# MihailMihov/simd-raytracer

Measured on AMD Instinct MI355X. Metric: Mrays/s (intersect invocations per second), hw09/scene5 dragon 1920x1080 1spp, higher is better.
Workload: dtype f32; 1 GPU; BASELINE configs[1]: scenes/hw09/scene5.crtscene 1920x1080 1spp max_ray_depth=5 (primary + shadow + reflection rays), kd_tree_simd_accel semantics; rays_per_frame=2726485, primary_rays=2073600, parallelism=bucket-tiles x1

## Files before the change

simd-raytracer_amd/csrc/accel.hpp:

```cpp
#pragma once

#include <hip/hip_runtime.h>

#include <cstdlib>
#include <mutex>
#include <string>
#include <vector>

#include "abi_guard.hpp"
#include "kernels.hpp"
#include "stream.hpp"
#include "build.hpp"
#include "dev_mem.hpp"
#include "frame_plan.hpp"
#include "update_plan.hpp"

struct rtk_knobs {
    uint32_t slice_min_tris = rtk::kSliceMinTrisDefault;
    bool shadow_exit = true;
    bool skip_unlit_shadow = true;
    bool bundle_cull = true;
    bool auto_trials = true;
    bool cost_feedback = true;
    unsigned resort_every = 16;
    uint32_t light_cycles = 140000u;
    uint32_t order_floor_cycles = 20000u;
    bool batch_scalar_surv = false;
    bool stream_scalar_surv = true;
    bool repack = true;
    bool raster_tiles = true;
    int repack_skip_bits = 6;
    bool repack_full_bounds = false;
    int repack_skip_bits2 = 14;
    bool repack_dirs3 = false;
    int repack_trace = -1;
    size_t group8_below = 9000;
    int stream_node_factor = 0;
    int stream_deep_level = 99, stream_deep_mode = RTK_TRACE_AUTO;
    uint32_t auto_min_lanes = 12;
    int stream_sort_from = -1;
    bool stream_debug = false;
    bool stream_side = true;
    int stream_lanes = 4;
    int stream_slices = 0;
    int stream_batch = 0;
    int stream_mem_gb = 96;
    int stream_side_below = 2;
    bool first_frame_prior = true;
    bool fast_occluders = true;
    bool camera_keeps_order = false;
    size_t views_launch_units = 131072;
    bool traversal_fast = false;
    size_t adaptive_chunk_pixels = size_t(1) << 20;

    static rtk_knobs from_env() {
        rtk_knobs k;
        auto geti = [](const char *name, long &out) { const char *e = std::getenv(name); if (!e || !*e) return false; out = std::atol(e); return true; };
        long v;
        if (geti("RTK_SLICE_MIN_TRIS", v) && v > 0) k.slice_min_tris = uint32_t(v);
        if (geti("RTK_SHADOW_EARLY_EXIT", v)) k.shadow_exit = v != 0;
        if (geti("RTK_SKIP_UNLIT_SHADOW", v)) k.skip_unlit_shadow = v != 0;
        if (geti("RTK_BUNDLE_CULL", v)) k.bundle_cull = v != 0;
        if (geti("RTK_AUTO_TRIALS", v)) k.auto_trials = v != 0;
        if (geti("RTK_COST_FEEDBACK", v)) k.cost_feedback = v != 0;
        if (geti("RTK_COST_RESORT_EVERY", v) && v > 0) k.resort_every = unsigned(v);
        if (geti("RTK_LIGHT_BELOW_CYCLES", v) && v >= 0) k.light_cycles = uint32_t(v);
        if (geti("RTK_ORDER_FLOOR_CYCLES", v) && v >= 0) k.order_floor_cycles = uint32_t(v);
        if (geti("RTK_REPACK", v)) k.repack = v != 0;
        if (geti("RTK_RASTER_TILES", v)) k.raster_tiles = v != 0;
        if (geti("RTK_REPACK_FULL_BOUNDS", v)) k.repack_full_bounds = v != 0;
        if (geti("RTK_REPACK_SKIP_BITS2", v) && v >= 0 && v <= 22) k.repack_skip_bits2 = int(v);
        if (geti("RTK_REPACK_DIRS3", v)) k.repack_dirs3 = v != 0;
        if (geti("RTK_REPACK_SKIP_BITS", v) && v >= 0 && v <= 14) k.repack_skip_bits = int(v);
        if (geti("RTK_STREAM_SCALAR_SURV", v)) k.stream_scalar_surv = v != 0;
        if (geti("RTK_BATCH_SCALAR_SURV", v)) k.batch_scalar_surv = v != 0;
        if (geti("RTK_REPACK_TRACE", v) && (v == RTK_TRACE_AUTO || v == RTK_TRACE_WAVE || v == RTK_TRACE_LANE)) k.repack_trace = int(v);
        if (geti("RTK_GROUP8_BELOW_BLOCKS", v) && v >= 0) k.group8_below = size_t(v);
        if (geti("RTK_STREAM_NODE_FACTOR", v) && v >= 1) k.stream_node_factor = int(v);
        if (geti("RTK_STREAM_DEEP_LEVEL", v)) k.stream_deep_level = int(v);
        if (geti("RTK_STREAM_DEEP_MODE", v)) k.stream_deep_mode = int(v);
        if (geti("RTK_AUTO_MIN_LANES", v) && v > 0 && v <= 64) k.auto_min_lanes = uint32_t(v);
        if (geti("RTK_STREAM_SORT_FROM", v)) k.stream_sort_from = int(v);
        if (geti("RTK_STREAM_DEBUG", v)) k.stream_debug = v != 0;
        if (geti("RTK_STREAM_SIDE", v)) k.stream_side = v != 0;
        if (geti("RTK_TRAVERSAL_FAST", v)) k.traversal_fast = v != 0;
        if (geti("RTK_FIRST_FRAME_PRIOR", v)) k.first_frame_prior = v != 0;
        if (geti("RTK_STREAM_SLICES", v) && (v == 0 || v == 1 || v == 2 || v == 4)) k.stream_slices = int(v);
        if (geti("RTK_STREAM_BATCH", v) && v >= 0 && v <= 4096) k.stream_batch = int(v);
        if (geti("RTK_STREAM_MEM_GB", v) && v >= 1 && v <= 256) k.stream_mem_gb = int(v);
        if (geti("RTK_FAST_OCCLUDERS", v)) k.fast_occluders = v != 0;
        if (geti("RTK_STREAM_SIDE_BELOW", v) && v >= 0) k.stream_side_below = int(v);
        if (geti("RTK_VIEWS_LAUNCH_UNITS", v) && v >= 1 && v <= (1l << 30)) k.views_launch_units = size_t(v);
        if (geti("RTK_CAMERA_KEEPS_ORDER", v)) k.camera_keeps_order = v != 0;
        if (geti("RTK_STREAM_LANES", v) && v >= 1 && v <= rtk::dev::kStreamLanes) k.stream_lanes = int(v);
        if (geti("RTK_ADAPTIVE_CHUNK_PIXELS", v) && v >= 1 && v <= (1l << 30)) k.adaptive_chunk_pixels = size_t(v);
        return k;
    }
};
// ... 246 lines not shown
    if (src.empty()) return RTK_OK;
    const hipError_t e = hipMemcpy(dst.get(), src.data(), src.size() * sizeof(T), hipMemcpyHostToDevice);
    if (e != hipSuccess) { dst.reset(); return hip_fail(e, "upload"); }
    return RTK_OK;
}

inline bool valid_mode(int m) { return m == RTK_TRACE_AUTO || m == RTK_TRACE_LANE || m == RTK_TRACE_WAVE; }
inline bool valid_batch_mode(int m) { return valid_mode(m) || m == RTK_TRACE_REPACK; }
inline bool valid_frame_mode(int m) { return valid_mode(m) || m == RTK_TRACE_GROUP4 || m == RTK_TRACE_GROUP8 || m == RTK_TRACE_GROUP16 ||
           m == RTK_TRACE_STREAM || m == RTK_TRACE_TWOPASS; }

inline int stream_slices_for(const HostTree &t) {
    double refs = 0.0, sq = 0.0;
    for (const DevNode &l : t.dev_leaves) { refs += double(l.b); sq += double(l.b) * double(l.b); }
    return (refs > 0.0 && sq / refs < 150.0) ? 1 : 4;
}

inline bool scene_forks(const rtk_accel *a, int diffuse_rays) { return a->has_refractive || diffuse_rays > 0; }
inline bool scene_general(const rtk_accel *a, int diffuse_rays) { return scene_forks(a, diffuse_rays) || !a->scene.textures.empty(); }

inline unsigned long long *counters_now(const rtk_accel *a) { return a->d_counters.get() + size_t(a->cnt.current) * kCounterAllocWords; }
inline unsigned long long *counters_other(const rtk_accel *a) { return a->d_counters.get() + size_t(a->cnt.current ^ 1) * kCounterAllocWords; }

int ensure_device(rtk_accel *a, hipStream_t s = nullptr);
dev::TreeView tree_view(const rtk_accel *a);
enum : unsigned { kKeepViewOrders = 1u, kKeepTrial = 2u };
inline void forget_orders(rtk_accel *a, unsigned keep = 0u) {
    a->fb.forget();
    a->cnt.forget();
    if (!(keep & kKeepViewOrders)) for (rtk_cost_feedback &f : a->fb_views) f.forget();
    for (rtk_cost_feedback &f : a->fb_regions) f.forget();
    if (!(keep & kKeepTrial)) a->trial.abandon();
}

int remake_occluders(rtk_accel *a, const std::vector<DevMaterial> &materials, const DevMaterial *d_materials, hipStream_t s);
int ensure_update_static(rtk_accel *a);
void dense_texture_slots(rtk_accel *a);
const std::vector<float> &host_vert_uv(rtk_accel *a);
int ensure_vert_uv_dev(rtk_accel *a);
int frame_geom(const rtk_accel *a, const rtk_render_params *p, FrameGeom &g);
rtk_view accel_camera(const rtk_accel *a);
void camera_args(const rtk_view &cam, const rtk_render_params *p, const FrameGeom &g, dev::RenderArgs &A);
int ensure_stream_ws(rtk_accel *a, size_t pixels, size_t nodes, size_t lights, bool need_sum, int lanes);
hipError_t zero_counters(rtk_accel *a, hipStream_t s);
void record_last(rtk_accel *a, hipStream_t s, bool stats, uint64_t primary);
int radiance_device_impl(rtk_accel *a, const rtk_ray *d_rays, const uint32_t *d_ids, size_t n, const rtk_radiance_params *p,
                         float *d_rgb, hipStream_t s, uint32_t *n_chunks_out);
void free_stream_ws(rtk_accel *a);
struct StreamSetup {
    dev::StreamArgs S;
    int deep_level, deep_mode, sort_from, slices;
    size_t factor, node_bytes, budget;
};
StreamSetup stream_args(const rtk_accel *a, const dev::RenderArgs &A, int diffuse_rays, bool forks);
int claim_stream_ws(rtk_accel *a, hipStream_t s);
int release_stream_ws(rtk_accel *a, hipStream_t s);
int fork_lanes(rtk_accel *a, int lanes, hipStream_t s);
int join_lanes(rtk_accel *a, int lanes, hipStream_t s);
dev::RenderArgs frame_args(const rtk_accel *a, const rtk_render_params *p, const FrameGeom &g, const rtk_view &cam, float *d_out);
int adaptive_device_impl(rtk_accel *a, const rtk_render_params *p, const rtk_adaptive_params *ap, const FrameGeom &g, float *d_rgb,
                         uint32_t *d_samples, float *d_noise, hipStream_t s);

}
```

simd-raytracer_amd/csrc/api_frame.hip:

```cpp
#include <cmath>
#include <cstdio>
#include <cstring>
#include <mutex>

#include "accel.hpp"
#include "stream_plan.hpp"

namespace rtk {

int frame_geom(const rtk_accel *a, const rtk_render_params *p, FrameGeom &g) {
    if (!a || !p) return fail(RTK_ERR_INVALID, "null accel or params");
    const int64_t w = p->width > 0 ? p->width : a->scene.width;
    const int64_t h = p->height > 0 ? p->height : a->scene.height;
    if (w <= 0 || h <= 0 || w > 65536 || h > 65536) return fail(RTK_ERR_INVALID, "image size must be in [1, 65536]");
    if (p->spp < 1) return fail(RTK_ERR_INVALID, "spp must be >= 1");
    if (p->max_ray_depth < 0 || p->max_ray_depth > kMaxRayDepth)
        return fail(RTK_ERR_INVALID, "max_ray_depth must be in [0, 16]");
    if (p->diffuse_rays < 0 || p->diffuse_rays > 32767) return fail(RTK_ERR_INVALID, "diffuse_rays must be in [0, 32767]");
    if (!valid_frame_mode(p->trace_mode)) return fail(RTK_ERR_INVALID, "unknown trace_mode");
    if (p->sample_begin < 0 || p->sample_count < 0 || p->sample_begin >= p->spp ||
        int64_t(p->sample_begin) + p->sample_count > p->spp)
        return fail(RTK_ERR_INVALID, "sample_begin / sample_count must select samples inside [0, spp)");
    if (p->sample_count == 0 && p->sample_begin != 0) return fail(RTK_ERR_INVALID, "sample_count == 0 means all samples: sample_begin must be 0");
    g.sample_begin = p->sample_begin;
// ... 283 lines not shown
    RTK_MEM(fb.cost.reserve(cap));
    RTK_MEM(fb.order.reserve(2 * (2 * cap + 4) + 8));
    RTK_MEM(fb.bins.reserve(cap));
    fb.state.units = cap;
    return RTK_OK;
}

struct ListSet { uint32_t *order, *hdr, *wg_list; };
ListSet list_set(rtk_cost_feedback &fb, int k, size_t units) {
    uint32_t *const order = fb.order.get() + size_t(k) * (2 * fb.state.units + 4);
    return {order, order + units, order + units + 4};
}

int launch_sort(rtk_accel *a, rtk_cost_feedback &fb, int k, int frame_mode, size_t units, hipStream_t s) {
    const ListSet L = list_set(fb, k, units);
    RTK_HIP_AS(launch_order_by_cost(fb.cost.get(), fb.bins.get(), L.order, L.wg_list, L.hdr, uint32_t(units),
                                    frame_mode == RTK_TRACE_GROUP4 ? a->knobs.light_cycles >> 4 : 0u, a->knobs.order_floor_cycles >> 4, 4u, s),
               "launch k_order_by_cost");
    RTK_MEM(fb.nwgs_host.reserve(1));
    RTK_MEM(fb.nwgs_ev.ensure());
    RTK_HIP(hipMemcpyAsync(fb.nwgs_host.get(), L.hdr, sizeof(uint32_t), hipMemcpyDeviceToHost, s));
    RTK_HIP(hipEventRecord(fb.nwgs_ev.get(), s));
    return RTK_OK;
}

int order_launch(rtk_accel *a, rtk_cost_feedback &fb, const rtk_render_params *p, const FrameGeom &g, dev::RenderArgs &A, int frame_mode,
                 size_t units, hipStream_t s, OrderState::Step &step) {
    uint64_t sig[5];
    shape_sig(g, p->spp, p->max_ray_depth, p->diffuse_rays, sig);
    sig[3] = (uint64_t(uint32_t(g.bucket)) << 32) | (uint64_t(uint32_t(g.sample_end - g.sample_begin) & 0xFFFFu) << 16) | uint32_t(p->trace_mode);
    sig[4] = A.regions ? ((1ull << 63) | (uint64_t(A.n_regions) << 32) | uint64_t(A.n_units))
                       : (A.views ? uint64_t(A.n_views) : 0ull);
    RTK_TRY(ensure_feedback_ws(a, fb, g, units));
    step = fb.state.step(sig, frame_mode, p->collect_stats != 0, A.regions != nullptr, {a->knobs.first_frame_prior, a->knobs.resort_every});
    const ListSet L = list_set(fb, step.read_set, units);
    if (step.prior)
        RTK_HIP_AS(launch_block_prior(A, fb.bins.get(), L.order, L.wg_list, L.hdr,
                                      reinterpret_cast<uint32_t *>(A.counters + kPriorScratchWord), 4u, s), "launch k_block_prior");
    if (step.sort_front) RTK_TRY(launch_sort(a, fb, step.read_set, frame_mode, units, s));
    if (step.use_order) { A.order_in = L.order; A.order_hdr = L.hdr; A.wg_list = L.wg_list; }
    if (&fb == &a->fb) a->cnt.after_order(step);
    A.cost_out = fb.cost.get();
    return RTK_OK;
}

int render_megakernel(rtk_accel *a, rtk_cost_feedback &fb, const rtk_render_params *p, const FrameGeom &g, dev::RenderArgs &A, bool general,
                      hipStream_t s) {
    const size_t units = A.regions ? size_t(A.n_units) : (A.views ? g.blocks() * A.n_views : g.blocks());
    A.n_units = uint32_t(units);
    const int frame_mode = OrderState::frame_mode(p->trace_mode, units, a->knobs.group8_below);
    OrderState::Step step = {};
    if (a->knobs.cost_feedback && units > 0 && units <= 0x7FFFFFFFull) {
        const int rc = order_launch(a, fb, p, g, A, frame_mode, units, s, step);
        if (rc != RTK_OK) { fb.forget(); return rc; }
    }
    unsigned n_wgs = 0;
    if (A.wg_list != nullptr) {
        bool ready = false;
        if (fb.state.awaits_count() && !(ready = hipEventQuery(fb.nwgs_ev.get()) == hipSuccess)) (void)hipGetLastError();
        n_wgs = fb.state.workgroups(ready, fb.nwgs_host.get());
    }
    int rc = RTK_OK;
    const hipError_t e = launch_render(A, frame_mode, p->collect_stats != 0, general, s, n_wgs);
    if (e != hipSuccess) rc = hip_fail(e, "launch k_render");
    if (rc == RTK_OK && step.sort_behind) rc = launch_sort(a, fb, step.write_set, frame_mode, units, s);
    if (rc != RTK_OK) fb.forget();
    return rc;
}

}

dev::RenderArgs frame_args(const rtk_accel *a, const rtk_render_params *p, const FrameGeom &g, const rtk_view &cam, float *d_out) {
    dev::RenderArgs A = scene_args(a, p->collect_stats);
    camera_args(cam, p, g, A);
    A.max_depth = p->max_ray_depth; A.diffuse_rays = p->diffuse_rays;
// ... 416 lines not shown
        if (ids) RTK_HIP(hipMemcpy(a->rad_ids.get(), ids, n * sizeof(uint32_t), hipMemcpyHostToDevice));
        uint32_t n_chunks = 0;
        RTK_TRY(radiance_device_impl(a, a->rad_rays.get(), ids ? a->rad_ids.get() : nullptr, n, p, a->rad_rgb.get(), nullptr, &n_chunks));
        RTK_HIP(hipMemcpy(rgb, a->rad_rgb.get(), n * 3 * sizeof(float), hipMemcpyDeviceToHost));
        unsigned long long h[kRadianceTotalWords] = {};
        RTK_HIP(hipMemcpy(h, a->d_rad_counters.get() + radiance_total_word(dev::kStreamLanes), sizeof(h), hipMemcpyDeviceToHost));
        if (counters) {
            std::memset(counters, 0, sizeof(*counters));
            counters->rays = h[kRadianceRays]; counters->primary = n;
        }
        if (a->knobs.stream_debug)
            std::fprintf(stderr, "[rtk radiance] rays %zu chunks %u redone %llu node_cap %u\n", n, n_chunks, h[kRadianceRedone], a->ws.node_cap);
        return RTK_OK;
    });
}


int rtk_accel_get_camera(const rtk_accel *a, rtk_view *out) {
    return abi_guard([&]() -> int {
        if (!a || !out) return fail(RTK_ERR_INVALID, "null accel or view");
        std::lock_guard<std::mutex> lock(const_cast<rtk_accel *>(a)->mu);
        *out = accel_camera(a);
        return RTK_OK;
    });
}

int rtk_accel_set_camera(rtk_accel *a, const rtk_view *view) {
    return abi_guard([&]() -> int {
        if (!a || !view) return fail(RTK_ERR_INVALID, "null accel or view");
        std::lock_guard<std::mutex> lock(a->mu);
        std::memcpy(a->scene.cam_pos, view->position, sizeof(a->scene.cam_pos));
        std::memcpy(a->scene.cam_mat, view->matrix, sizeof(a->scene.cam_mat));
        if (!a->knobs.camera_keeps_order) forget_orders(a, kKeepViewOrders | kKeepTrial);
        return RTK_OK;
    });
}

int rtk_render_views_device(rtk_accel *a, const rtk_render_params *p, const rtk_view *d_views, int32_t n_views, float *d_out, void *stream) {
    return abi_guard([&]() -> int {
        if (!a || !p) return fail(RTK_ERR_INVALID, "null accel or params");
        FrameGeom g;
        RTK_TRY(views_check(a, p, d_views, n_views, d_out, g));
        if (n_views == 0) return RTK_OK;
        std::lock_guard<std::mutex> lock(a->mu);
        RTK_TRY(ensure_device(a, static_cast<hipStream_t>(stream)));
        return render_views_impl(a, p, g, nullptr, d_views, n_views, d_out, static_cast<hipStream_t>(stream));
    });
}

int rtk_render_views(rtk_accel *a, const rtk_render_params *p, const rtk_view *views, int32_t n_views, float *rgb, rtk_counters *counters) {
    return abi_guard([&]() -> int {
        if (!a || !p) return fail(RTK_ERR_INVALID, "null accel or params");
        FrameGeom g;
        RTK_TRY(views_check(a, p, views, n_views, rgb, g));
        if (n_views == 0) return RTK_OK;
        {
            std::lock_guard<std::mutex> lock(a->mu);
            RTK_TRY(ensure_device(a));
            const size_t n = size_t(n_views), nf = n * g.width * g.height * 3;
            RTK_MEM(a->views_tab.reserve(n));
            RTK_MEM(a->views_out.reserve(nf));
            RTK_HIP(hipMemcpy(a->views_tab.get(), views, n * sizeof(rtk_view), hipMemcpyHostToDevice));
            if (p->sample_begin > 0) RTK_HIP(hipMemcpy(a->views_out.get(), rgb, nf * sizeof(float), hipMemcpyHostToDevice));
            RTK_TRY(render_views_impl(a, p, g, views, a->views_tab.get(), n_views, a->views_out.get(), nullptr));
            RTK_HIP(hipMemcpy(rgb, a->views_out.get(), nf * sizeof(float), hipMemcpyDeviceToHost));
        }
// ... 79 lines not shown
```

simd-raytracer_amd/csrc/api_state.hip:

```cpp
#include <algorithm>
#include <cstring>
#include <mutex>

#include "accel.hpp"

using namespace rtk;

namespace {

int reserve_lights(rtk_accel *a, size_t n) {
    if (n <= a->d_lights.capacity()) return RTK_OK;
    DevBuf<DevLight> larger;
    RTK_MEM(larger.reserve(n, grow_lights()));
    a->d_lights.swap(larger);
    return RTK_OK;
}

void lights_changed(rtk_accel *a, size_t n_before) {
    if (a->scene.lights.size() == n_before) return;
    forget_orders(a, kKeepTrial);
}


constexpr size_t kTexelLimit = 0x7FFFFFFFull;
constexpr size_t kSlotAlign = 16;

inline size_t slot_round(size_t bytes) { return (bytes + kSlotAlign - 1) & ~(kSlotAlign - 1); }
inline bool is_bitmap(const DevTexture &t) { return t.kind == RTK_TEX_BITMAP; }
inline size_t texel_bytes(const DevTexture &t) { return is_bitmap(t) ? size_t(t.bmp[0]) * size_t(t.bmp[1]) * 3 : 0; }

inline bool bitmap_size_ok(int32_t w, int32_t h) { return w >= 1 && h >= 1 && int64_t(w) * int64_t(h) <= (int64_t{1} << 28); }

void host_tri_uv(const rtk_accel *a, const std::vector<float> &vert_uv, std::vector<DevTriUv> &out) {
    std::vector<size_t> first(a->mesh_nverts.size() + 1, 0);
    for (size_t mi = 0; mi < a->mesh_nverts.size(); ++mi) first[mi + 1] = first[mi] + size_t(a->mesh_nverts[mi]);
    out.resize(a->tree.triangles.size());
    for (size_t i = 0; i < out.size(); ++i) {
        const HostTriangle &tr = a->tree.triangles[i];
        for (int k = 0; k < 3; ++k) {
            const size_t g = first[tr.mesh] + tr.vi[k];
            out[i].uv[k * 2] = vert_uv[g * 2]; out[i].uv[k * 2 + 1] = vert_uv[g * 2 + 1];
        }
    }
}

int make_tri_uv(rtk_accel *a, hipStream_t s) {
    RTK_TRY(ensure_update_static(a));
    const size_t nt = size_t(a->scene.n_triangles);
    RTK_MEM(a->topo_spare.tri_uv.reserve(std::max<size_t>(1, nt), grow_bytes()));
    RTK_HIP_AS(launch_tri_uv(a->topo.index.get(), a->topo_vert_uv.get(), uint32_t(nt), uint32_t(a->scene.n_vertices), a->topo_spare.tri_uv.get(), s),
               "launch k_tri_uv");
    return RTK_OK;
// ... 67 lines not shown
struct HostTexels {
    bool same = false;
    std::vector<DevTexture> table;
    std::vector<uint8_t> pixels;
};
int host_texels(const rtk_accel *a, size_t texture, int32_t w, int32_t h, const uint8_t *rgb, HostTexels &H) {
    const std::vector<DevTexture> &tex = a->scene.textures;
    const size_t was = texel_bytes(tex[texture]), need = size_t(w) * size_t(h) * 3, at = size_t(tex[texture].bmp[2]);
    const std::vector<uint8_t> &old = a->scene.tex_pixels;
    if (old.size() - was + need > kTexelLimit) return fail(RTK_ERR_INVALID, "the texel bytes of all bitmaps must fit an int32 offset");
    H.same = tex[texture].bmp[0] == w && tex[texture].bmp[1] == h;
    if (H.same) return RTK_OK;
    H.table = tex;
    H.table[texture].bmp[0] = w; H.table[texture].bmp[1] = h;
    for (size_t i = 0; i < tex.size(); ++i)
        if (is_bitmap(tex[i]) && size_t(tex[i].bmp[2]) > at) H.table[i].bmp[2] = int32_t(size_t(tex[i].bmp[2]) - was + need);
    H.pixels.resize(old.size() - was + need);
    std::memcpy(H.pixels.data(), old.data(), at);
    if (rgb) std::memcpy(H.pixels.data() + at, rgb, need);
    std::memcpy(H.pixels.data() + at + need, old.data() + at + was, old.size() - at - was);
    return RTK_OK;
}

int check_texel_call(const rtk_accel *a, int32_t texture, int32_t w, int32_t h) {
    if (texture < 0 || size_t(texture) >= a->scene.textures.size()) return fail(RTK_ERR_INVALID, "texture index out of range");
    if (!bitmap_size_ok(w, h)) return fail(RTK_ERR_INVALID, "bad bitmap texture size");
    if (!is_bitmap(a->scene.textures[size_t(texture)])) return fail(RTK_ERR_INVALID, "the texture is not a bitmap");
    return RTK_OK;
}

void adopt_texels(rtk_accel *a, size_t texture, HostTexels &H, const uint8_t *rgb, TexelPlan *P, bool on_device) {
    if (H.same) { if (rgb) std::memcpy(a->scene.tex_pixels.data() + a->scene.textures[texture].bmp[2], rgb, texel_bytes(a->scene.textures[texture])); }
    else { a->scene.textures.swap(H.table); a->scene.tex_pixels.swap(H.pixels); }
    if (!P) return;
    if (P->moved) { a->d_tex_pixels.swap(a->tx_pixels); a->d_textures.swap(a->tx_textures); }
    a->tx_slots.swap(P->slots); a->tx_used = P->used;
    a->tx_slots[texture].on_device = on_device;
}

template <typename Write>
int set_texels_device(rtk_accel *a, int32_t texture, int32_t w, int32_t h, const void *d_src, hipStream_t s, Write write) {
    if (!a || !d_src) return fail(RTK_ERR_INVALID, "null accel or texels");
    std::lock_guard<std::mutex> lock(a->mu);
    RTK_TRY(check_texel_call(a, texture, w, h));
    HostTexels H;
    RTK_TRY(host_texels(a, size_t(texture), w, h, nullptr, H));
    RTK_TRY(ensure_device(a));
    RTK_HIP(a->geom_fence.quiesce());
    DevTexture row = a->scene.textures[size_t(texture)];
    row.bmp[0] = w; row.bmp[1] = h;
    TexelPlan P;
    RTK_TRY(place_texels(a, size_t(texture), row, size_t(w) * size_t(h) * 3, s, P));
    RTK_TRY(write(P.dst, s));
    RTK_HIP(a->geom_fence.publish(s));
    adopt_texels(a, size_t(texture), H, nullptr, &P, true);
    return RTK_OK;
}

}

void rtk::dense_texture_slots(rtk_accel *a) {
    const std::vector<DevTexture> &tex = a->scene.textures;
    a->tx_slots.assign(tex.size(), rtk_accel::TexSlot{});
    for (size_t i = 0; i < tex.size(); ++i)
        if (is_bitmap(tex[i])) { a->tx_slots[i].off = tex[i].bmp[2]; a->tx_slots[i].cap = texel_bytes(tex[i]); }
    a->tx_used = a->scene.tex_pixels.size();
// ... 106 lines not shown
                if (m.texture < 0 || size_t(m.texture) >= a->scene.textures.size()) return fail(RTK_ERR_INVALID, "texture material refers to a texture that does not exist");
            } else m.texture = -1;
            m.pad = 0u;
        }
        if (a->on_device) {
            RTK_HIP(hipSetDevice(a->device));
            RTK_HIP(a->geom_fence.quiesce());
            RTK_MEM(a->st_materials.reserve(table.size()));
            if (!table.empty()) RTK_HIP(hipMemcpy(a->st_materials.get(), table.data(), table.size() * sizeof(DevMaterial), hipMemcpyHostToDevice));
            RTK_TRY(remake_occluders(a, table, a->st_materials.get(), nullptr));
            a->d_materials.swap(a->st_materials);
        }
        a->scene.materials.swap(table);
        a->has_refractive = any_refractive(a->scene.materials);
        forget_orders(a);
        return RTK_OK;
    });
}

int rtk_accel_get_background(const rtk_accel *a, float rgb[3]) {
    return abi_guard([&]() -> int {
        if (!a || !rgb) return fail(RTK_ERR_INVALID, "null accel or colour");
        std::lock_guard<std::mutex> lock(const_cast<rtk_accel *>(a)->mu);
        std::memcpy(rgb, a->scene.background, sizeof(a->scene.background));
        return RTK_OK;
    });
}

int rtk_accel_set_background(rtk_accel *a, const float rgb[3]) {
    return abi_guard([&]() -> int {
        if (!a || !rgb) return fail(RTK_ERR_INVALID, "null accel or colour");
        std::lock_guard<std::mutex> lock(a->mu);
        std::memcpy(a->scene.background, rgb, sizeof(a->scene.background));
        return RTK_OK;
    });
}


int rtk_accel_get_textures(const rtk_accel *a, rtk_texture *out, int32_t cap, int32_t *n) {
    return abi_guard([&]() -> int {
        if (!a || !n) return fail(RTK_ERR_INVALID, "null accel or count");
        std::lock_guard<std::mutex> lock(const_cast<rtk_accel *>(a)->mu);
        const std::vector<DevTexture> &tex = a->scene.textures;
        *n = int32_t(tex.size());
        const size_t take = (out && cap > 0) ? std::min(tex.size(), size_t(cap)) : 0;
        for (size_t i = 0; i < take; ++i) {
            rtk_texture t{};
            t.kind = tex[i].kind;
            if (is_bitmap(tex[i])) { t.width = tex[i].bmp[0]; t.height = tex[i].bmp[1]; }
            else { std::memcpy(t.color_a, tex[i].a, sizeof(t.color_a)); std::memcpy(t.color_b, tex[i].b, sizeof(t.color_b)); t.param = tex[i].param; }
            out[i] = t;
        }
        return RTK_OK;
    });
}

int rtk_accel_get_texture_pixels(const rtk_accel *a, int32_t texture, uint8_t *out, size_t cap, size_t *n_bytes) {
    return abi_guard([&]() -> int {
        if (!a || !n_bytes) return fail(RTK_ERR_INVALID, "null accel or size");
        std::lock_guard<std::mutex> lock(const_cast<rtk_accel *>(a)->mu);
        if (texture < 0 || size_t(texture) >= a->scene.textures.size()) return fail(RTK_ERR_INVALID, "texture index out of range");
        const DevTexture &t = a->scene.textures[size_t(texture)];
        *n_bytes = texel_bytes(t);
        const size_t take = out ? std::min(*n_bytes, cap) : 0;
        if (take == 0) return RTK_OK;
        if (a->on_device && a->tx_slots[size_t(texture)].on_device) {
// ... 36 lines not shown
            if (is_bitmap(table[i])) std::memcpy(texels.data() + table[i].bmp[2], pixels[i], texel_bytes(table[i]));
        const bool first = a->scene.textures.empty() && !table.empty();
        std::vector<DevTriUv> tri_uv;
        std::vector<rtk_accel::TexSlot> slots(table.size());
        size_t used = 0;
        if (a->on_device) {
            RTK_HIP(hipSetDevice(a->device));
            RTK_HIP(a->geom_fence.quiesce());
            std::vector<DevTexture> rows(table.size());
            for (size_t i = 0; i < table.size(); ++i) {
                if (is_bitmap(table[i])) { slots[i].off = int32_t(used); slots[i].cap = slot_round(texel_bytes(table[i])); used += slots[i].cap; }
                if (used > kTexelLimit) return fail(RTK_ERR_INVALID, "the texel bytes of all bitmaps must fit an int32 offset");
                rows[i] = device_row(table[i], slots[i]);
            }
            RTK_MEM(a->tx_textures.reserve(std::max<size_t>(1, rows.size())));
            if (!rows.empty()) RTK_HIP(hipMemcpy(a->tx_textures.get(), rows.data(), rows.size() * sizeof(DevTexture), hipMemcpyHostToDevice));
            if (used > 0) RTK_MEM(a->tx_pixels.reserve(used, grow_bytes()));
            for (size_t i = 0; i < table.size(); ++i)
                if (is_bitmap(table[i])) RTK_HIP(hipMemcpy(a->tx_pixels.get() + slots[i].off, pixels[i], texel_bytes(table[i]), hipMemcpyHostToDevice));
            if (first) {
                RTK_TRY(ensure_vert_uv_dev(a));
                RTK_TRY(make_tri_uv(a, nullptr));
                RTK_HIP(a->geom_fence.publish(nullptr));
            }
        } else if (first) host_tri_uv(a, host_vert_uv(a), tri_uv);
        if (a->on_device) {
            a->d_textures.swap(a->tx_textures);
            if (used > 0) a->d_tex_pixels.swap(a->tx_pixels);
            if (first) a->topo.tri_uv.swap(a->topo_spare.tri_uv);
            a->tx_slots.swap(slots); a->tx_used = used;
        } else if (first) a->tree.dev_tri_uv.swap(tri_uv);
        a->scene.textures.swap(table);
        a->scene.tex_pixels.swap(texels);
        return RTK_OK;
    });
}

int rtk_accel_set_texture_pixels(rtk_accel *a, int32_t texture, int32_t width, int32_t height, const uint8_t *rgb) {
    return abi_guard([&]() -> int {
        if (!a || !rgb) return fail(RTK_ERR_INVALID, "null accel or texels");
        std::lock_guard<std::mutex> lock(a->mu);
        RTK_TRY(check_texel_call(a, texture, width, height));
        HostTexels H;
        RTK_TRY(host_texels(a, size_t(texture), width, height, rgb, H));
        if (!a->on_device) { adopt_texels(a, size_t(texture), H, rgb, nullptr, false); return RTK_OK; }
        RTK_HIP(hipSetDevice(a->device));
        RTK_HIP(a->geom_fence.quiesce());
        DevTexture row = a->scene.textures[size_t(texture)];
        row.bmp[0] = width; row.bmp[1] = height;
        const size_t need = size_t(width) * size_t(height) * 3;
        TexelPlan P;
        RTK_TRY(place_texels(a, size_t(texture), row, need, nullptr, P));
        RTK_HIP(hipMemcpy(P.dst, rgb, need, hipMemcpyHostToDevice));
        RTK_HIP(hipStreamSynchronize(nullptr));
        adopt_texels(a, size_t(texture), H, rgb, &P, false);
        return RTK_OK;
    });
}

int rtk_accel_set_texture_pixels_device(rtk_accel *a, int32_t texture, int32_t width, int32_t height, const uint8_t *d_rgb, void *hip_stream) {
    return abi_guard([&]() -> int {
        const size_t need = size_t(width) * size_t(height) * 3;
        return set_texels_device(a, texture, width, height, d_rgb, static_cast<hipStream_t>(hip_stream), [&](uint8_t *dst, hipStream_t s) -> int {
            RTK_HIP(hipMemcpyAsync(dst, d_rgb, need, hipMemcpyDeviceToDevice, s));
            return RTK_OK;
        });
// ... 21 lines not shown
            RTK_HIP(hipSetDevice(a->device));
            RTK_HIP(hipDeviceSynchronize());
            RTK_HIP(hipMemcpy(uvs, a->topo_vert_uv.get(), n * sizeof(float), hipMemcpyDeviceToHost));
        } else std::memcpy(uvs, host_vert_uv(w).data(), n * sizeof(float));
        return RTK_OK;
    });
}

int rtk_accel_set_uvs(rtk_accel *a, const float *uvs) {
    return abi_guard([&]() -> int {
        if (!a || !uvs) return fail(RTK_ERR_INVALID, "null accel or uvs");
        std::lock_guard<std::mutex> lock(a->mu);
        const size_t n = size_t(a->scene.n_vertices) * 2;
        std::vector<float> uv(uvs, uvs + n);
        const bool textured = !a->scene.textures.empty();
        std::vector<DevTriUv> tri_uv;
        if (a->on_device) {
            RTK_HIP(hipSetDevice(a->device));
            RTK_HIP(a->geom_fence.quiesce());
            RTK_MEM(a->topo_vert_uv.reserve(std::max<size_t>(2, n)));
            a->vert_uv_dev = false;
            if (n > 0) RTK_HIP(hipMemcpy(a->topo_vert_uv.get(), uv.data(), n * sizeof(float), hipMemcpyHostToDevice));
            if (textured) {
                RTK_TRY(make_tri_uv(a, nullptr));
                RTK_HIP(a->geom_fence.publish(nullptr));
                a->topo.tri_uv.swap(a->topo_spare.tri_uv);
            }
            a->vert_uv_dev = true;
        } else if (textured) host_tri_uv(a, uv, tri_uv);
        if (!a->on_device && textured) a->tree.dev_tri_uv.swap(tri_uv);
        a->vert_uv.swap(uv);
        a->vert_uv_made = true;
        a->uvs_on_device = false;
        return RTK_OK;
    });
}

int rtk_accel_set_uvs_device(rtk_accel *a, const float *d_uvs, void *hip_stream) {
    return abi_guard([&]() -> int {
        if (!a || !d_uvs) return fail(RTK_ERR_INVALID, "null accel or uvs");
        std::lock_guard<std::mutex> lock(a->mu);
        hipStream_t s = static_cast<hipStream_t>(hip_stream);
        RTK_TRY(ensure_device(a));
        RTK_HIP(a->geom_fence.quiesce());
        const size_t n = size_t(a->scene.n_vertices) * 2;
        const bool textured = !a->scene.textures.empty();
        RTK_MEM(a->topo_vert_uv.reserve(std::max<size_t>(2, n)));
        if (textured) RTK_TRY(ensure_update_static(a));
        a->vert_uv_dev = false;
        if (n > 0) RTK_HIP(hipMemcpyAsync(a->topo_vert_uv.get(), d_uvs, n * sizeof(float), hipMemcpyDeviceToDevice, s));
        if (textured) RTK_TRY(make_tri_uv(a, s));
        RTK_HIP(a->geom_fence.publish(s));
        if (textured) a->topo.tri_uv.swap(a->topo_spare.tri_uv);
        a->vert_uv_dev = true;
        a->uvs_on_device = true;
        return RTK_OK;
    });
}

}
```

simd-raytracer_amd/csrc/frame_plan.hpp:

```cpp
#pragma once

#include <cstddef>
#include <cstdint>
#include <cstring>

#include "../../include/rtk.h"

namespace rtk {

struct FrameGeom {
    uint32_t width, height, bucket, tiles_x, tiles_y, n_buckets, blocks_side, buckets_per_rank;
    uint32_t skew_q;
    int rank, world;
    int sample_begin, sample_end;
    uint64_t blocks_of(uint64_t buckets) const { return buckets * blocks_side * blocks_side; }
    size_t blocks() const { return size_t(blocks_of(buckets_per_rank)); }
};

inline void shape_sig(const FrameGeom &g, int spp, int max_ray_depth, int diffuse_rays, uint64_t out[3]) {
    out[0] = (uint64_t(uint32_t(g.width)) << 32) | uint32_t(g.height);
    out[1] = (uint64_t(uint32_t(g.rank)) << 32) | uint32_t(g.world);
    out[2] = (uint64_t(uint32_t(spp)) << 32) | (uint64_t(uint32_t(max_ray_depth)) << 16) | uint32_t(diffuse_rays);
}

struct EngineTrial {
    enum { kNoRecord = -1, kPipelinePair = 0, kMegakernelPair = 2 };
    struct Step { bool stream; int record; };
    uint64_t sig[3] = {0, 0, 0};
    int state = 0;

    static bool applies(int trace_mode, bool forks, bool stats) { return trace_mode == RTK_TRACE_AUTO && forks && !stats; }
    bool same(const uint64_t s[3]) const { return std::memcmp(s, sig, sizeof(sig)) == 0; }
    bool waiting(const uint64_t s[3]) const { return state == 3 && same(s); }
    void verdict(float t_stream, float t_mega) { state = t_mega < t_stream ? 5 : 4; }
    void abandon() { state = 0; }
    Step next(const uint64_t s[3], bool trials_on) {
        if (!same(s)) { std::memcpy(sig, s, sizeof(sig)); state = 0; }
        if (!trials_on) return {true, kNoRecord};
        switch (state) {
            case 0: state = 1; return {true, kPipelinePair};
            case 1: state = 2; return {false, kNoRecord};
            case 2: state = 3; return {false, kMegakernelPair};
            case 5: return {false, kNoRecord};
            default: return {true, kNoRecord};
        }
    }
};

struct OrderState {
    struct Knobs { bool first_frame_prior; unsigned resort_every; };
    struct Step { bool prior, resort, use_order, sort_front, sort_behind; int read_set, write_set; };
    size_t units = 0;
    uint64_t sig[5] = {0, 0, 0, 0, 0};
    bool valid = false;
    bool order_valid = false;
    unsigned age = 0;
    bool nwgs_pending = false, nwgs_known = false;
    int set = 0;
    bool presorted = false;

    void forget() { valid = false; order_valid = false; age = 0; nwgs_pending = false; nwgs_known = false; set = 0; presorted = false; }

    static int frame_mode(int trace_mode, size_t n_units, size_t group8_below) {
        if (trace_mode == RTK_TRACE_TWOPASS) return RTK_TRACE_GROUP4;
        return trace_mode != RTK_TRACE_AUTO ? trace_mode : (n_units < group8_below ? RTK_TRACE_GROUP8 : RTK_TRACE_GROUP4);
    }

    size_t capacity(size_t n_units, bool is_frame_table, uint64_t native) {
        if (units >= n_units) return units;
        size_t cap = n_units;
        if (is_frame_table && units == 0 && native > cap && native <= (1ull << 24)) cap = size_t(native);
        units = 0; valid = false; order_valid = false;
        return cap;
    }

    Step step(const uint64_t s[5], int mode, bool stats, bool regions, const Knobs &k) {
        const bool same_shape = valid && std::memcmp(s, sig, sizeof(sig)) == 0;
        if (!same_shape) { order_valid = false; set = 0; presorted = false; }
        Step r = {!same_shape && k.first_frame_prior && mode == RTK_TRACE_GROUP4 && !stats && !regions, false, false, false, false, 0, 0};
        if (same_shape) {
            r.resort = !order_valid || age >= k.resort_every;
            if (r.resort) {
                r.sort_front = !presorted;
                if (presorted) set ^= 1;
                presorted = false;
                order_valid = true; age = 0; nwgs_known = false; nwgs_pending = true;
            }
            age += 1;
            r.sort_behind = age >= k.resort_every;
            presorted = r.sort_behind;
        }
        r.use_order = r.prior || same_shape;
        r.read_set = set; r.write_set = set ^ 1;
        std::memcpy(sig, s, sizeof(sig));
        valid = true;
        return r;
    }

    bool awaits_count() const { return order_valid && nwgs_pending; }
    unsigned workgroups(bool ready, const uint32_t *host_word) {
        if (!order_valid) return 0;
        if (nwgs_pending && ready) { nwgs_pending = false; nwgs_known = true; }
        return nwgs_known && !nwgs_pending ? *host_word : 0;
    }
};

struct CounterState {
    struct Step { int current; bool fill, carry; };
    int current = 0;
    bool other_zero = false;
    const void *stream = nullptr;

    void forget() { other_zero = false; }
    void after_order(const OrderState::Step &st) { if (st.prior || !st.use_order) forget(); }
    Step frame(const void *s, bool carries) {
        const bool flip = carries && other_zero && stream == s;
        if (flip) current ^= 1;
        other_zero = carries; stream = s;
        return {current, !flip, carries};
    }
};

// ... 29 lines not shown
```

simd-raytracer_amd/csrc/kernels.hip:

```cpp
#include <hip/hip_runtime.h>

#include "kernels.hpp"
#include "trace.hip.hpp"
#include "shade.hip.hpp"

namespace rtk {
namespace dev {

template <int MODE, bool STATS, bool LDS_NODES>
__global__ __launch_bounds__(256) void k_intersect(IntersectArgs A) {
    extern __shared__ __attribute__((aligned(16))) unsigned char smem[];
    DevNode *lds_nodes = reinterpret_cast<DevNode *>(smem);
    if (LDS_NODES) stage_nodes(A.tree.nodes, A.tree.n_nodes, lds_nodes);

    const size_t slot = (size_t)blockIdx.x * blockDim.x + threadIdx.x;
    const bool active = slot < A.n;
    size_t i = (active && A.perm != nullptr) ? (size_t)A.perm[slot] : slot;
    uint32_t raster_w = A.raster_w;
    if (A.verdict != nullptr) {
        if (A.verdict[16] != 0u) return;
        raster_w = A.verdict[15];
        if (raster_w < 64u || (raster_w & 7u) != 0u || (size_t)raster_w * 16u > A.n) raster_w = 0u;
    }
    if (raster_w != 0u) {
// ... 540 lines not shown
                                    if (res.y != 0.0f) acc = acc + (res.x * albedo);
                                    more_rays += fl & 1u;
                                }
                            }
                            light_k += 1;
                        }
                    }
                }
            } else if (!hit) {
                ret = (pend == PEND_CHILD_BG) ? background : black;
                state = ST_RETURN;
            } else {
                const Surface s = reconstruct(A.tree, cand);
                P = ray.o + (cand.t * ray.d);
                hn = s.hit_normal; fn = s.face_normal; din = ray.d;
                hit_tri = s.tri; hit_mat = s.material;
                if (FORKS && A.tri_uv != nullptr && A.materials[hit_mat].kind == RTK_MAT_TEXTURE)
                    albedo = sample_texture(A.textures + A.materials[hit_mat].texture, A.tri_uv + hit_tri, cand.u, cand.v, A.tex_pixels);
                state = ST_SHADE;
            }
        }
        nrays_wave += (uint32_t)__popcll(__builtin_amdgcn_ballot_w64((more_rays & 1u) != 0u)) +
                      2u * (uint32_t)__popcll(__builtin_amdgcn_ballot_w64((more_rays & 2u) != 0u)) +
                      4u * (uint32_t)__popcll(__builtin_amdgcn_ballot_w64((more_rays & 4u) != 0u)) +
                      8u * (uint32_t)__popcll(__builtin_amdgcn_ballot_w64((more_rays & 8u) != 0u));
        static_assert(kBurstMaxJobs + 1u <= 15u, "a lane's rays of one iteration fit four bits");
    }

    const uint32_t lane = fresh_lane();
    if (kPhases && valid && writer) {
        const Pixel p = my_pixel();
        phases.write(sx.probe(), lane, view_out() + pixel_slot(p) * 3);
    }
    if (A.cost_out != nullptr && lane == 0u && gwave < A.n_units) {
        const unsigned long long dt = (__builtin_readcyclecounter() - cost_t0) >> (light ? 5 : 4);
        A.cost_out[gwave] = dt > 0xFFFFFFFFull ? 0xFFFFFFFFu : (uint32_t)dt;
    }
    {
        const unsigned long long dt = __builtin_amdgcn_s_memrealtime() - real_t0;
        if (lane == 0u && dt >= kCriticalMinTicks) atomicMax(A.counters + kCriticalWord + (gwave % (uint32_t)kRayCounterShards), dt);
    }
    if (SLICES > 1 && !light) group_post_exit(group_sh);
    const uint32_t total = nrays_wave;
    if (STATS && writer) flush_stats(st, 0u, A.counters);
    if (lane == 0u && writer) atomicAdd(A.counters + kRayShardWord + (gwave % (uint32_t)kRayCounterShards), (unsigned long long)total);
}

__global__ __launch_bounds__(256) void k_assemble(AssembleArgs A) {
    const size_t i = (size_t)blockIdx.x * blockDim.x + threadIdx.x;
    if (i >= (size_t)A.width * A.height) return;
    const uint32_t px = (uint32_t)(i % A.width), py = (uint32_t)(i / A.width);
    const uint32_t bucket = (py / A.bucket) * A.tiles_x + (px / A.bucket);
    uint32_t rank, local;
    bucket_owner(bucket, A.tiles_x, A.world, A.skew_q, rank, local);
    const size_t src = (((size_t)rank * A.buckets_per_rank + local) * A.bucket + (py % A.bucket)) * A.bucket + (px % A.bucket);
    A.rgb[i * 3 + 0] = A.gathered[src * 3 + 0];
    A.rgb[i * 3 + 1] = A.gathered[src * 3 + 1];
    A.rgb[i * 3 + 2] = A.gathered[src * 3 + 2];
}

__global__ __launch_bounds__(256) void k_camera_rays(RenderArgs A, int sample, rtk_ray *out) {
    const size_t i = (size_t)blockIdx.x * blockDim.x + threadIdx.x;
    if (i >= (size_t)A.width * A.height) return;
    const uint32_t px = (uint32_t)(i % A.width), py = (uint32_t)(i / A.width);
    const Ray r = camera_ray(A, px, py, root_key(pcg_hash(A.seed), py * A.width + px, (uint32_t)sample));
    float *o = reinterpret_cast<float *>(out + i);
    o[0] = r.o.x; o[1] = r.o.y; o[2] = r.o.z; o[3] = r.d.x; o[4] = r.d.y; o[5] = r.d.z;
}

// ... 434 lines not shown
```

simd-raytracer_amd/csrc/kernels.hpp:

```cpp
#pragma once

#include <hip/hip_runtime.h>

#include "rtk_internal.hpp"
#include "counters.hpp"

namespace rtk {

constexpr int kMaxRayDepth = 16;
constexpr unsigned long long kCriticalMinTicks = 1000;
constexpr uint32_t kSliceMinTrisDefault = 33;
constexpr size_t kMaxNodeLdsBytes = 48 * 1024;

}

#include "trace.hip.hpp"
#include "regions_plan.hpp"

namespace rtk {
namespace dev {

__host__ __device__ inline uint32_t rank_bucket(uint32_t rank, uint32_t local, uint32_t world, uint32_t skew_q) {
    if (skew_q == 0u) return rank + local * world;
    const uint32_t by = local / skew_q, m = local % skew_q;
// ... 20 lines not shown

struct RenderArgs {
    TreeView tree;
    const DevMaterial *materials;
    const DevTexture *textures;
    const DevTriUv *tri_uv;
    const uint8_t *tex_pixels;
    const DevLight *lights;
    int n_lights;
    int has_refractive;
    float cam_pos[3];
    float cam_mat[9];
    float background[3];
    uint32_t width, height;
    float aspect;
    float tan_half_fov;
    int spp, max_depth, diffuse_rays;
    int sample_begin, sample_end;
    uint32_t seed;
    float shadow_bias, reflection_bias, refraction_bias;
    uint32_t bucket, tiles_x, tiles_y, n_buckets, blocks_per_bucket_side;
    uint32_t buckets_per_rank;
    uint32_t skew_q;
    int rank, world;
    uint32_t slice_min_tris;
    int compact;
    float *out;
    unsigned long long *counters;
    unsigned long long *zero_next;
    unsigned long long keep_offsets_[5];
    const uint32_t *only_if;
    uint32_t n_units;
    uint32_t *cost_out;
    float width_f, height_f, spp_f, gi_div_f;
    const uint32_t *order_in;
    const uint32_t *order_hdr;
    const uint32_t *wg_list;
    int shadow_exit;
    int skip_unlit;
    int occl_on;
    TreeView occl;
    const float *views;
    uint32_t n_views, units_per_view;
    size_t view_stride;
    const RegionEntry *regions;
    uint32_t n_regions;

    __device__ __forceinline__ size_t out_index(uint32_t local_bucket, uint32_t lx, uint32_t ly, uint32_t px,
                                                uint32_t py) const {
        return compact ? (((size_t)local_bucket * bucket + ly) * bucket + lx) : ((size_t)py * width + px);
    }
};

struct AssembleArgs {
    const float *gathered;
    float *rgb;
    uint32_t width, height, bucket, tiles_x, world, buckets_per_rank, skew_q;
};

}

hipError_t launch_intersect(const dev::IntersectArgs &A, int mode, bool stats, hipStream_t s);
hipError_t launch_render(const dev::RenderArgs &A, int mode, bool stats, bool forks, hipStream_t s, unsigned n_workgroups = 0);
hipError_t launch_order_by_cost(const uint32_t *cost, uint8_t *bins , uint32_t *order, uint32_t *wg_list ,
                                uint32_t *hdr , uint32_t n, uint32_t light_below, uint32_t floor_below, uint32_t pack,
                                hipStream_t s);
// ... 13 lines not shown
```

simd-raytracer_amd/csrc/phases.hip.hpp:

```cpp
#pragma once

#include <hip/hip_runtime.h>

#include <cstdint>

namespace rtk {
namespace dev {

enum PhaseSlot : int {
    PH_TOTAL = 0,
    PH_TRACE, PH_N_TRACE,
    PH_STEPS,
    PH_N_SMALL, PH_T_SMALL, PH_C_SMALL,
    PH_N_BIG, PH_T_BIG, PH_C_BIG,
    PH_PROLOGUE, PH_TO_FIRST_TRACE, PH_FIRST_TRACE, PH_AFTER_FIRST_TRACE,
    PH_CHUNKS, PH_SURV, PH_CTRIS,
    PH_RT0, PH_RT1,
    PH_WG,
    PH_WAIT,
    PH_TR0, PH_TR1, PH_TR2, PH_TR3, PH_TR4, PH_TR5,
    PH_KIND0, PH_KIND1, PH_KIND2, PH_KIND3, PH_KIND4, PH_KIND5,
    PH_C_BUND, PH_C_LIST,
    PH_OWN,
    PH_STG_N,
    PH_STG_W1, PH_STG_L1, PH_STG_W2, PH_STG_L2, PH_STG_W3, PH_STG_L3,
    PH_STG_L4,
    PH_SLOTS
};

#ifdef RTK_DEBUG_PHASES
constexpr bool kPhases = true;
#define RTK_PHASES_ONLY(...) __VA_ARGS__
#else
constexpr bool kPhases = false;
#define RTK_PHASES_ONLY(...)
#endif

struct PhaseTallies { uint32_t v[PH_SLOTS] = {}; };
struct Stamp {
    RTK_PHASES_ONLY(unsigned long long t0;)
// ... 20 lines not shown

struct FrameProbe {
    RTK_PHASES_ONLY(unsigned long long entry, rt0, begin = 0, first_trace = 0, after_first = 0, tr0 = 0, w0 = 0;)
    static __device__ __forceinline__ FrameProbe enter() { return FrameProbe{RTK_PHASES_ONLY(__builtin_readcyclecounter(), __builtin_amdgcn_s_memrealtime())}; }
    __device__ __forceinline__ void prologue_done() { RTK_PHASES_ONLY(begin = __builtin_readcyclecounter();) }
    __device__ __forceinline__ void trace_begins() { RTK_PHASES_ONLY(tr0 = __builtin_readcyclecounter(); if (first_trace == 0) first_trace = tr0;) }
    __device__ __forceinline__ void trace_returned() { RTK_PHASES_ONLY(w0 = __builtin_readcyclecounter();) }
    __device__ __forceinline__ void trace_done(const Probe p, const bool burst, const bool sliced, const uint32_t burst_plog, const bool in_root) {
        RTK_PHASES_ONLY(
        p.since(Stamp{w0}, PH_WAIT);
        if (burst && sliced) p.t->v[PH_OWN] = (uint32_t)(w0 - tr0);
        for (int i = 0; i < 6; ++i) if (p.t->v[PH_N_TRACE] == (uint32_t)i) {
            p.t->v[PH_TR0 + i] = (uint32_t)(__builtin_readcyclecounter() - tr0);
            p.t->v[PH_KIND0 + i] = burst ? 100u + burst_plog : (uint32_t)__popcll(__builtin_amdgcn_ballot_w64(in_root));
        }
        p.since(Stamp{tr0}, PH_TRACE); p.add(PH_N_TRACE, 1u);
        if (after_first == 0) after_first = __builtin_readcyclecounter();)
    }
    __device__ __forceinline__ void write(const Probe p, const uint32_t lane, float *o) const {
        RTK_PHASES_ONLY(
        const unsigned long long now = __builtin_readcyclecounter(), rt1 = __builtin_amdgcn_s_memrealtime();
        float vals[PH_SLOTS];
        for (int i = 0; i < PH_SLOTS; ++i) vals[i] = (float)p.t->v[i];
        vals[PH_TOTAL] = (float)(now - begin);
        vals[PH_PROLOGUE] = (float)(begin - entry);
        vals[PH_TO_FIRST_TRACE] = (float)(first_trace - begin);
        vals[PH_FIRST_TRACE] = (float)(after_first - first_trace);
        vals[PH_AFTER_FIRST_TRACE] = (float)(now - after_first);
        vals[PH_RT0] = (float)(rt0 & 0xFFFFFFull);
        vals[PH_RT1] = (float)(rt1 & 0xFFFFFFull);
        vals[PH_WG] = (float)blockIdx.x;
        float v = 0.f;
        for (int i = 0; i < PH_SLOTS; ++i) v = (lane == (uint32_t)i) ? vals[i] : v;
        o[0] = v; o[1] = 0.f; o[2] = 0.f;)
    }
};

}
}
```

Baseline: 14570 Mrays/s.

## Back off cost-feedback resort interval and blend per-wave cost measurements

Adds exponential backoff to the cost-feedback resort schedule. The resort interval doubles after each resort, up to a configurable cap, and restarts when lights, textures, UVs, background or camera change. Per-wave cycle costs are now blended into the previous table as an exponential moving average, flagged through the low bit of the cost pointer. The aim is to spend less time on sort launches for static scenes while keeping the orders stable, at the risk of stale orderings. The phase probe also records the XCC and hardware ID in debug builds.

After: 14710 Mrays/s (median of 5 runs). About the same (+0.9%).

```diff
diff --git a/simd-raytracer_amd/csrc/accel.hpp b/simd-raytracer_amd/csrc/accel.hpp
--- a/simd-raytracer_amd/csrc/accel.hpp
+++ b/simd-raytracer_amd/csrc/accel.hpp
@@ -23,6 +23,7 @@
     bool auto_trials = true;
     bool cost_feedback = true;
     unsigned resort_every = 16;
+    unsigned resort_max = 256;
     uint32_t light_cycles = 140000u;
     uint32_t order_floor_cycles = 20000u;
     bool batch_scalar_surv = false;
@@ -64,6 +65,7 @@
         if (geti("RTK_AUTO_TRIALS", v)) k.auto_trials = v != 0;
         if (geti("RTK_COST_FEEDBACK", v)) k.cost_feedback = v != 0;
         if (geti("RTK_COST_RESORT_EVERY", v) && v > 0) k.resort_every = unsigned(v);
+        if (geti("RTK_COST_RESORT_MAX", v) && v >= 0 && v <= (1l << 20)) k.resort_max = unsigned(v);
         if (geti("RTK_LIGHT_BELOW_CYCLES", v) && v >= 0) k.light_cycles = uint32_t(v);
         if (geti("RTK_ORDER_FLOOR_CYCLES", v) && v >= 0) k.order_floor_cycles = uint32_t(v);
         if (geti("RTK_REPACK", v)) k.repack = v != 0;
@@ -376,6 +378,11 @@
     for (rtk_cost_feedback &f : a->fb_regions) f.forget();
     if (!(keep & kKeepTrial)) a->trial.abandon();
 }
+inline void restart_resort_backoff(rtk_accel *a) {
+    a->fb.state.restart_backoff();
+    for (rtk_cost_feedback &f : a->fb_views) f.state.restart_backoff();
+    for (rtk_cost_feedback &f : a->fb_regions) f.state.restart_backoff();
+}
 
 int remake_occluders(rtk_accel *a, const std::vector<DevMaterial> &materials, const DevMaterial *d_materials, hipStream_t s);
 int ensure_update_static(rtk_accel *a);
diff --git a/simd-raytracer_amd/csrc/api_frame.hip b/simd-raytracer_amd/csrc/api_frame.hip
--- a/simd-raytracer_amd/csrc/api_frame.hip
+++ b/simd-raytracer_amd/csrc/api_frame.hip
@@ -339,6 +339,7 @@
     sig[4] = A.regions ? ((1ull << 63) | (uint64_t(A.n_regions) << 32) | uint64_t(A.n_units))
                        : (A.views ? uint64_t(A.n_views) : 0ull);
     RTK_TRY(ensure_feedback_ws(a, fb, g, units));
+    fb.state.resort_cap = a->knobs.resort_max;
     step = fb.state.step(sig, frame_mode, p->collect_stats != 0, A.regions != nullptr, {a->knobs.first_frame_prior, a->knobs.resort_every});
     const ListSet L = list_set(fb, step.read_set, units);
     if (step.prior)
@@ -347,7 +348,7 @@
     if (step.sort_front) RTK_TRY(launch_sort(a, fb, step.read_set, frame_mode, units, s));
     if (step.use_order) { A.order_in = L.order; A.order_hdr = L.hdr; A.wg_list = L.wg_list; }
     if (&fb == &a->fb) a->cnt.after_order(step);
-    A.cost_out = fb.cost.get();
+    A.cost_out = dev::RenderArgs::with_blend(fb.cost.get(), step.blend);
     return RTK_OK;
 }
 
@@ -830,6 +831,7 @@
         std::memcpy(a->scene.cam_pos, view->position, sizeof(a->scene.cam_pos));
         std::memcpy(a->scene.cam_mat, view->matrix, sizeof(a->scene.cam_mat));
         if (!a->knobs.camera_keeps_order) forget_orders(a, kKeepViewOrders | kKeepTrial);
+        else restart_resort_backoff(a);
         return RTK_OK;
     });
 }
diff --git a/simd-raytracer_amd/csrc/api_state.hip b/simd-raytracer_amd/csrc/api_state.hip
--- a/simd-raytracer_amd/csrc/api_state.hip
+++ b/simd-raytracer_amd/csrc/api_state.hip
@@ -17,7 +17,7 @@
 }
 
 void lights_changed(rtk_accel *a, size_t n_before) {
-    if (a->scene.lights.size() == n_before) return;
+    if (a->scene.lights.size() == n_before) { restart_resort_backoff(a); return; }
     forget_orders(a, kKeepTrial);
 }
 
@@ -151,6 +151,7 @@
 void adopt_texels(rtk_accel *a, size_t texture, HostTexels &H, const uint8_t *rgb, TexelPlan *P, bool on_device) {
     if (H.same) { if (rgb) std::memcpy(a->scene.tex_pixels.data() + a->scene.textures[texture].bmp[2], rgb, texel_bytes(a->scene.textures[texture])); }
     else { a->scene.textures.swap(H.table); a->scene.tex_pixels.swap(H.pixels); }
+    restart_resort_backoff(a);
     if (!P) return;
     if (P->moved) { a->d_tex_pixels.swap(a->tx_pixels); a->d_textures.swap(a->tx_textures); }
     a->tx_slots.swap(P->slots); a->tx_used = P->used;
@@ -323,6 +324,7 @@
         if (!a || !rgb) return fail(RTK_ERR_INVALID, "null accel or colour");
         std::lock_guard<std::mutex> lock(a->mu);
         std::memcpy(a->scene.background, rgb, sizeof(a->scene.background));
+        restart_resort_backoff(a);
         return RTK_OK;
     });
 }
@@ -425,6 +427,7 @@
         } else if (first) a->tree.dev_tri_uv.swap(tri_uv);
         a->scene.textures.swap(table);
         a->scene.tex_pixels.swap(texels);
+        restart_resort_backoff(a);
         return RTK_OK;
     });
 }
@@ -512,6 +515,7 @@
         a->vert_uv.swap(uv);
         a->vert_uv_made = true;
         a->uvs_on_device = false;
+        restart_resort_backoff(a);
         return RTK_OK;
     });
 }
@@ -534,8 +538,9 @@
         if (textured) a->topo.tri_uv.swap(a->topo_spare.tri_uv);
         a->vert_uv_dev = true;
         a->uvs_on_device = true;
-        return RTK_OK;
-    });
-}
-
-}
+        restart_resort_backoff(a);
+        return RTK_OK;
+    });
+}
+
+}
diff --git a/simd-raytracer_amd/csrc/frame_plan.hpp b/simd-raytracer_amd/csrc/frame_plan.hpp
--- a/simd-raytracer_amd/csrc/frame_plan.hpp
+++ b/simd-raytracer_amd/csrc/frame_plan.hpp
@@ -49,7 +49,7 @@
 
 struct OrderState {
     struct Knobs { bool first_frame_prior; unsigned resort_every; };
-    struct Step { bool prior, resort, use_order, sort_front, sort_behind; int read_set, write_set; };
+    struct Step { bool prior, resort, use_order, sort_front, sort_behind; int read_set, write_set; bool blend; };
     size_t units = 0;
     uint64_t sig[5] = {0, 0, 0, 0, 0};
     bool valid = false;
@@ -58,8 +58,19 @@
     bool nwgs_pending = false, nwgs_known = false;
     int set = 0;
     bool presorted = false;
+    unsigned resort_cap = 0;
+    unsigned interval = 0;
+    bool hold_interval = false;
 
-    void forget() { valid = false; order_valid = false; age = 0; nwgs_pending = false; nwgs_known = false; set = 0; presorted = false; }
+    void forget() {
+        valid = false; order_valid = false; age = 0; nwgs_pending = false; nwgs_known = false; set = 0; presorted = false;
+        interval = 0; hold_interval = false;
+    }
+    void restart_backoff() {
+        interval = 0;
+        if (presorted) hold_interval = true; else age = 0;
+    }
+    unsigned every(const Knobs &k) const { return k.resort_every > 1 && interval > k.resort_every ? interval : k.resort_every; }
 
     static int frame_mode(int trace_mode, size_t n_units, size_t group8_below) {
         if (trace_mode == RTK_TRACE_TWOPASS) return RTK_TRACE_GROUP4;
@@ -76,18 +87,22 @@
 
     Step step(const uint64_t s[5], int mode, bool stats, bool regions, const Knobs &k) {
         const bool same_shape = valid && std::memcmp(s, sig, sizeof(sig)) == 0;
-        if (!same_shape) { order_valid = false; set = 0; presorted = false; }
-        Step r = {!same_shape && k.first_frame_prior && mode == RTK_TRACE_GROUP4 && !stats && !regions, false, false, false, false, 0, 0};
+        if (!same_shape) { order_valid = false; set = 0; presorted = false; interval = 0; hold_interval = false; }
+        Step r = {!same_shape && k.first_frame_prior && mode == RTK_TRACE_GROUP4 && !stats && !regions, false, false, false, false, 0, 0, false};
         if (same_shape) {
-            r.resort = !order_valid || age >= k.resort_every;
+            r.blend = k.resort_every > 1 && resort_cap > k.resort_every;
+            r.resort = !order_valid || age >= every(k);
             if (r.resort) {
+                const unsigned twice = every(k) > resort_cap / 2 ? resort_cap : 2 * every(k);
+                interval = (order_valid && !hold_interval && k.resort_every > 1 && twice > k.resort_every) ? twice : 0;
+                hold_interval = false;
                 r.sort_front = !presorted;
                 if (presorted) set ^= 1;
                 presorted = false;
                 order_valid = true; age = 0; nwgs_known = false; nwgs_pending = true;
             }
             age += 1;
-            r.sort_behind = age >= k.resort_every;
+            r.sort_behind = age >= every(k);
             presorted = r.sort_behind;
         }
         r.use_order = r.prior || same_shape;
diff --git a/simd-raytracer_amd/csrc/kernels.hip b/simd-raytracer_amd/csrc/kernels.hip
--- a/simd-raytracer_amd/csrc/kernels.hip
+++ b/simd-raytracer_amd/csrc/kernels.hip
@@ -596,9 +596,13 @@
         const Pixel p = my_pixel();
         phases.write(sx.probe(), lane, view_out() + pixel_slot(p) * 3);
     }
-    if (A.cost_out != nullptr && lane == 0u && gwave < A.n_units) {
+    const uintptr_t cost_word = (uintptr_t)A.cost_out;
+    uint32_t *const cost_table = (uint32_t *)(cost_word & ~(uintptr_t)1);
+    if (cost_table != nullptr && lane == 0u && gwave < A.n_units) {
         const unsigned long long dt = (__builtin_readcyclecounter() - cost_t0) >> (light ? 5 : 4);
-        A.cost_out[gwave] = dt > 0xFFFFFFFFull ? 0xFFFFFFFFu : (uint32_t)dt;
+        uint32_t cost = dt > 0xFFFFFFFFull ? 0xFFFFFFFFu : (uint32_t)dt;
+        if ((cost_word & 1u) != 0u) { const uint32_t old = cost_table[gwave]; cost = old - (old >> 2) + (cost >> 2); }
+        cost_table[gwave] = cost;
     }
     {
         const unsigned long long dt = __builtin_amdgcn_s_memrealtime() - real_t0;
diff --git a/simd-raytracer_amd/csrc/kernels.hpp b/simd-raytracer_amd/csrc/kernels.hpp
--- a/simd-raytracer_amd/csrc/kernels.hpp
+++ b/simd-raytracer_amd/csrc/kernels.hpp
@@ -76,6 +76,7 @@
     const uint32_t *only_if;
     uint32_t n_units;
     uint32_t *cost_out;
+    __host__ __device__ static uint32_t *with_blend(uint32_t *table, bool blend) { return (uint32_t *)((uintptr_t)table | (blend ? 1u : 0u)); }
     float width_f, height_f, spp_f, gi_div_f;
     const uint32_t *order_in;
     const uint32_t *order_hdr;
diff --git a/simd-raytracer_amd/csrc/phases.hip.hpp b/simd-raytracer_amd/csrc/phases.hip.hpp
--- a/simd-raytracer_amd/csrc/phases.hip.hpp
+++ b/simd-raytracer_amd/csrc/phases.hip.hpp
@@ -6,6 +6,11 @@
 
 namespace rtk {
 namespace dev {
+
+constexpr int kGetregHwId = 4 | (0 << 6) | (31 << 11);
+constexpr int kGetregXccId = 20 | (0 << 6) | (3 << 11);
+__device__ __forceinline__ uint32_t hw_simd(const uint32_t hw_id) { return (hw_id >> 4) & 3u; }
+__device__ __forceinline__ uint32_t hw_cu_code(const uint32_t hw_id) { return (hw_id >> 8) & 0xFFu; }
 
 enum PhaseSlot : int {
     PH_TOTAL = 0,
@@ -92,7 +97,8 @@
         vals[PH_WG] = (float)blockIdx.x;
         float v = 0.f;
         for (int i = 0; i < PH_SLOTS; ++i) v = (lane == (uint32_t)i) ? vals[i] : v;
-        o[0] = v; o[1] = 0.f; o[2] = 0.f;)
+        const uint32_t place = ((__builtin_amdgcn_s_getreg(kGetregXccId) & 7u) << 16) | (__builtin_amdgcn_s_getreg(kGetregHwId) & 0xFFFFu);
+        o[0] = v; o[1] = (float)place; o[2] = 0.f;)
     }
 };
 
```
